# spartan-array/spartan

Hardware: AMD Instinct MI355X
Metric: spartan.dot TFLOP/s (+ map/reduce HBM GB/s) (higher is better)
Workload: dtype f32

## Files before the change

### spartan_amd/csrc/gemm_split.hpp

```cpp
#pragma once

typedef __bf16 gs_bf16x8 __attribute__((ext_vector_type(8)));
typedef __bf16 gs_bf16x4 __attribute__((ext_vector_type(4)));

namespace {

constexpr int GS_BK = 16;
constexpr int GS_RB = GS_BK * 2;
constexpr int GS_WN = 4;
constexpr unsigned GS_WIN_LO = (127u - 40u) << 23;
constexpr unsigned GS_WIN_HI = (127u + 40u) << 23;
constexpr size_t GS_IMAGE_CAP = (size_t)2 << 30;
constexpr size_t GS_WS_HEAD = 512;

template <int WN>
struct GsCfg {
  static constexpr int BM = 256, BN = 64 * WN, NW = 2 * WN, THREADS = 64 * NW;
  static constexpr int A_BYTES = BM * GS_RB, B_BYTES = BN * GS_RB;
  static constexpr int STAGE_BYTES = 3 * A_BYTES + 3 * B_BYTES;
  static constexpr int SMEM_BYTES = 2 * STAGE_BYTES;
  static constexpr int APW = A_BYTES / 1024 / NW, BPW = B_BYTES / 1024 / NW;
  static constexpr int NPIECES = 3 * APW + 3 * BPW;
  static constexpr int SLOTS = SP_CUS * (WN == 4 ? 1 : 2);
  static_assert(APW >= 1 && BPW >= 1 && APW * NW * 1024 == A_BYTES && BPW * NW * 1024 == B_BYTES, "tile / waves mismatch");
  static_assert(NPIECES * 4 <= 48, "one piece after every fourth MFMA");
};

__device__ __forceinline__ bool gs_outside(float v) {
  const unsigned b = __float_as_uint(v) & 0x7fffffffu;
  return b != 0u && (b < GS_WIN_LO || b >= GS_WIN_HI);
}

__device__ __forceinline__ void gs_cut(float v, __bf16& h, __bf16& m, __bf16& l) {
  h = (__bf16)v;
  const float r1 = v - (float)h;
  m = (__bf16)r1;
  l = (__bf16)(r1 - (float)m);
}

__device__ __forceinline__ void gs_raise(bool bad, unsigned* flag) {
  if (__any(bad) && (threadIdx.x & 63) == 0) atomicOr(flag, 1u);
}

__global__ __launch_bounds__(256) void sp_gemm_cut_rows_kernel(const float* __restrict__ A, int64_t lda, int M, int K,
                                                               __bf16* __restrict__ Ah, int64_t img,
                                                               unsigned* __restrict__ flag) {
  const int q = threadIdx.x & 7, row = blockIdx.x * 32 + (threadIdx.x >> 3);
  const int kpad = (K + GS_BK - 1) / GS_BK * GS_BK;
  bool bad = false;
  if (row < M) {
    const float* __restrict__ a = A + (int64_t)row * lda;
#pragma unroll
    for (int it = 0; it < 8; ++it) {
      const int k = blockIdx.y * 256 + it * 32 + 4 * q;
      if (k >= kpad) break;
      f32x4 v = {0.f, 0.f, 0.f, 0.f};
      if (k + 4 <= K) {
        v = *(const f32x4*)(a + k);
      } else {
#pragma unroll
        for (int e = 0; e < 4; ++e)
          if (k + e < K) v[e] = a[k + e];
      }
      gs_bf16x4 h, m, l;
#pragma unroll
      for (int e = 0; e < 4; ++e) {
        bad |= gs_outside(v[e]);
        __bf16 hh, mm, ll;
        gs_cut(v[e], hh, mm, ll);
        h[e] = hh;
        m[e] = mm;
        l[e] = ll;
      }
      const int64_t at = ((int64_t)(k >> 4) * M + row) * GS_BK + (k & 15);
      *(gs_bf16x4*)(Ah + at) = h;
      *(gs_bf16x4*)(Ah + img + at) = m;
      *(gs_bf16x4*)(Ah + 2 * img + at) = l;
    }
  }
  gs_raise(bad, flag);
}

__global__ __launch_bounds__(256) void sp_gemm_cut_cols_kernel(const float* __restrict__ B, int64_t ldb, int N, int K,
                                                               __bf16* __restrict__ Bh, int64_t img,
                                                               unsigned* __restrict__ flag) {
  __shared__ __attribute__((aligned(16))) __bf16 s[3][256 * GS_BK];
  const int n0 = blockIdx.x * 256, col = n0 + threadIdx.x, k0 = blockIdx.y * GS_BK;
  float v[GS_BK];
#pragma unroll
  for (int e = 0; e < GS_BK; ++e) v[e] = (col < N && k0 + e < K) ? B[(int64_t)(k0 + e) * ldb + col] : 0.f;
  bool bad = false;
  gs_bf16x8 h[2], m[2], l[2];
#pragma unroll
  for (int e = 0; e < GS_BK; ++e) {
    bad |= gs_outside(v[e]);
    __bf16 hh, mm, ll;
    gs_cut(v[e], hh, mm, ll);
    h[e >> 3][e & 7] = hh;
    m[e >> 3][e & 7] = mm;
    l[e >> 3][e & 7] = ll;
  }
#pragma unroll
  for (int c = 0; c < 2; ++c) {
    *(gs_bf16x8*)(&s[0][threadIdx.x * GS_BK + 8 * c]) = h[c];
    *(gs_bf16x8*)(&s[1][threadIdx.x * GS_BK + 8 * c]) = m[c];
    *(gs_bf16x8*)(&s[2][threadIdx.x * GS_BK + 8 * c]) = l[c];
  }
  __syncthreads();
  const int64_t base = ((int64_t)blockIdx.y * N + n0) * GS_BK;
#pragma unroll
  for (int p = 0; p < 3; ++p)
#pragma unroll
    for (int c = 0; c < 2; ++c) {
      const int at = (c * 256 + threadIdx.x) * 8;
      if (n0 + at / GS_BK < N) *(gs_bf16x8*)(Bh + p * img + base + at) = *(const gs_bf16x8*)(&s[p][at]);
    }
  gs_raise(bad, flag);
}

template <int WN>
__global__ __launch_bounds__(GsCfg<WN>::THREADS, 2) void sp_gemm_glds_kernel_bf16x3(
    const char* __restrict__ Ah, int64_t a_img, const char* __restrict__ Bh, int64_t b_img, float* __restrict__ C,
    int64_t ldc, int M, int N, int KT, int accumulate, int tiles_m, int tiles_n, int64_t a_slab, int64_t b_slab,
    const unsigned* __restrict__ flag_a, const unsigned* __restrict__ flag_b) {
  using G = GsCfg<WN>;
  constexpr int APW = G::APW, BPW = G::BPW, NPIECES = G::NPIECES;
  extern __shared__ __attribute__((aligned(16))) char gs_smem[];
  if ((*flag_a | *flag_b) != 0u) return;
  int tm, tn;
  sp_gemm_tile_of_block(blockIdx.x, gridDim.x, tiles_m, tiles_n, tm, tn);
  const int m0 = tm * G::BM, n0 = tn * G::BN;
  const int tid = threadIdx.x, lane = tid & 63;
  const int wid = __builtin_amdgcn_readfirstlane(tid >> 6);
  const int wm = wid / WN, wn = wid % WN;
  const int l31 = lane & 31, lh = lane >> 5;

  unsigned a_off[APW], b_off[BPW];
#pragma unroll
  for (int j = 0; j < APW; ++j) {
    const int slot = (wid * APW + j) * 64 + lane;
    int row = slot >> 1;
    const int q = (slot & 1) ^ ((row >> 4) & 1);
    if (m0 + row > M - 1) row = M - 1 - m0;
    a_off[j] = (unsigned)(row * GS_RB + q * 16);
  }
#pragma unroll
  for (int j = 0; j < BPW; ++j) {
    const int slot = (wid * BPW + j) * 64 + lane;
    int row = slot >> 1;
    const int q = (slot & 1) ^ ((row >> 4) & 1);
    if (n0 + row > N - 1) row = N - 1 - n0;
    b_off[j] = (unsigned)(row * GS_RB + q * 16);
  }
  const char* __restrict__ Ablk = Ah + (int64_t)m0 * GS_RB;
  const char* __restrict__ Bblk = Bh + (int64_t)n0 * GS_RB;
  const unsigned s_base = SP_LDS_ADDR(gs_smem);

#define GS_PIECE(i)                                                                                    \
  do {                                                                                                 \
    if ((i) < 3 * APW) {                                                                               \
      const int p_ = (i) / APW, j_ = (i) % APW;                                                        \
      SP_GLDS_S(Ablk + p_ * a_img + ka_, a_off[j_], st_ + p_ * G::A_BYTES + (wid * APW + j_) * 1024);  \
    } else {                                                                                           \
      const int p_ = ((i) - 3 * APW) / BPW, j_ = ((i) - 3 * APW) % BPW;                                \
      SP_GLDS_S(Bblk + p_ * b_img + kb_, b_off[j_],                                                    \
                st_ + 3 * G::A_BYTES + p_ * G::B_BYTES + (wid * BPW + j_) * 1024);                     \
    }                                                                                                  \
  } while (0)

  f32x16 acc[4][2];
#pragma unroll
  for (int i = 0; i < 4; ++i)
#pragma unroll
    for (int j = 0; j < 2; ++j)
#pragma unroll
      for (int r = 0; r < 16; ++r) acc[i][j][r] = 0.f;

  {
    const int64_t ka_ = 0, kb_ = 0;
    const unsigned st_ = s_base;
#pragma unroll
    for (int i = 0; i < NPIECES; ++i) GS_PIECE(i);
  }
  SP_GLDS_LANDED();
  __syncthreads();

  const int fslot = (lh ^ ((l31 >> 4) & 1)) * 16;
  const int a_frag = (wm * 128 + l31) * GS_RB + fslot;
  const int b_frag = 3 * G::A_BYTES + (wn * 64 + l31) * GS_RB + fslot;

  for (int t = 0; t < KT; ++t) {
    const bool more = t + 1 < KT;
    const int64_t ka_ = (int64_t)(t + 1) * a_slab, kb_ = (int64_t)(t + 1) * b_slab;
    const unsigned st_ = s_base + (unsigned)((t + 1) & 1) * G::STAGE_BYTES;
    const char* st = gs_smem + (t & 1) * G::STAGE_BYTES;
    gs_bf16x8 af[3][4], bf[3][2];
#pragma unroll
    for (int p = 0; p < 3; ++p) {
#pragma unroll
      for (int i = 0; i < 4; ++i) af[p][i] = *(const gs_bf16x8*)(st + p * G::A_BYTES + a_frag + i * 32 * GS_RB);
#pragma unroll
      for (int j = 0; j < 2; ++j) bf[p][j] = *(const gs_bf16x8*)(st + p * G::B_BYTES + b_frag + j * 32 * GS_RB);
    }
    int piece = 0;
#pragma unroll
    for (int idx = 0; idx < 48; ++idx) {
      const int term = idx >> 3, i = (idx & 7) >> 1, j = idx & 1;
      const int pa = term == 0 ? 2 : (term == 2 || term == 3) ? 1 : 0;
      const int pb = term == 1 ? 2 : (term == 2 || term == 4) ? 1 : 0;
      acc[i][j] = __builtin_amdgcn_mfma_f32_32x32x16_bf16(af[pa][i], bf[pb][j], acc[i][j], 0, 0, 0);
      if (idx % 4 == 3 && piece < NPIECES) {
        __builtin_amdgcn_sched_barrier(0);
        if (more) GS_PIECE(piece);
        __builtin_amdgcn_sched_barrier(0);
        ++piece;
      }
    }
    if (more) SP_GLDS_LANDED();
    __syncthreads();
  }
#undef GS_PIECE

#pragma unroll
  for (int i = 0; i < 4; ++i) {
#pragma unroll
    for (int j = 0; j < 2; ++j) {
      const int col = n0 + wn * 64 + j * 32 + l31;
#pragma unroll
      for (int r = 0; r < 16; ++r) {
        const int row = m0 + wm * 128 + i * 32 + (r & 3) + 8 * (r >> 2) + 4 * lh;
        if (row < M && col < N) {
          float* p = C + (int64_t)row * ldc + col;
          float v = acc[i][j][r];
          if (accumulate) v += *p;
          *p = v;
        }
      }
    }
  }
}

template <typename Cfg, int BM, int BN, int WM, int WN, int WGS>
__global__ __launch_bounds__(Cfg::THREADS, WGS) void sp_gemm_f32_gated_kernel(
    const float* __restrict__ A, int64_t lda, const float* __restrict__ B, int64_t ldb, float* __restrict__ C,
    int64_t ldc, int M, int N, int K, int accumulate, int tiles_m, int tiles_n, const unsigned* __restrict__ flag_a,
    const unsigned* __restrict__ flag_b) {
  if ((*flag_a | *flag_b) == 0u) return;
  sp_gemm_glds_body<Cfg, BM, BN, WM, WN>(A, lda, B, ldb, C, ldc, M, N, K, accumulate, tiles_m, tiles_n);
}

#define GS_CUT_BYTES_PER_S 3.0e12
#define GS_ISSUED_FLOPS 1.1e15
static bool sp_gemm_bf16_plan(int64_t M, int64_t N, int64_t K) {
  static int mode = -2;
  if (mode == -2) {
    const char* e = getenv("SP_GEMM_SPLIT");
    mode = e ? atoi(e) : 1;
  }
  using G = GsCfg<GS_WN>;
  if (mode == 0 || K < 16 || N % 4 != 0 || N < 4 || M < 1 || M > 2147483647LL || N > 2147483647LL || K > 2147483647LL)
    return false;
  const int64_t tb = ((M + 255) / 256) * ((N + 127) / 128);
  if (tb < 2 * SP_CUS || tb >= 2147483647LL) return false;
  double dp_cost;
  if (sp_gemm_dp_choice(M, N, &dp_cost) != 6 || sp_sk_plan(M, N, K)) return false;
  const int64_t KT = (K + GS_BK - 1) / GS_BK;
  if ((double)KT * 3.0 * GS_RB * ((double)M + (double)N) > (double)GS_IMAGE_CAP) return false;
  const double fp32_s = dp_cost * 128.0 * 128.0 * (double)K * 2.0 / (157.3e12 * 0.95 / SP_CUS);
  const int64_t tiles = ((M + G::BM - 1) / G::BM) * ((N + G::BN - 1) / G::BN);
  const int64_t rounds = (tiles + G::SLOTS - 1) / G::SLOTS;
  const double main_s = (double)rounds * G::SLOTS * (6.0 * 2.0 * G::BM * G::BN * (double)K) / GS_ISSUED_FLOPS;
  const double cut_s = 10.0 * ((double)M + (double)N) * (double)K / GS_CUT_BYTES_PER_S;
  return (main_s + cut_s + 20e-6) < 0.92 * fp32_s;
}

static size_t sp_gemm_bf16_ws_bytes(int64_t M, int64_t N, int64_t K) {
  return GS_WS_HEAD + (size_t)((K + GS_BK - 1) / GS_BK) * 3 * GS_RB * (size_t)(M + N);
}

constexpr size_t GS_IMG_HEAD = 256;

static size_t sp_gemm_bf16_image_bytes(int64_t rows, int64_t K) {
  return GS_IMG_HEAD + (size_t)((K + GS_BK - 1) / GS_BK) * 3 * GS_RB * (size_t)rows;
}

static long long gs_cut_launches = 0;

static void sp_gemm_bf16_cut(int side, const float* X, int64_t ld, int64_t rows, int64_t K, char* img, unsigned* flag,
                             hipStream_t st) {
  const int64_t KT = (K + GS_BK - 1) / GS_BK;
  const int64_t img_stride = KT * rows * GS_RB;
  __atomic_add_fetch(&gs_cut_launches, 1, __ATOMIC_RELAXED);
  if (side == 0)
    hipLaunchKernelGGL(sp_gemm_cut_rows_kernel, dim3((unsigned)((rows + 31) / 32), (unsigned)((K + 255) / 256)), dim3(256), 0,
                       st, X, ld, (int)rows, (int)K, (__bf16*)img, img_stride / 2, flag);
  else
    hipLaunchKernelGGL(sp_gemm_cut_cols_kernel, dim3((unsigned)((rows + 255) / 256), (unsigned)KT), dim3(256), 0, st, X, ld,
                       (int)rows, (int)K, (__bf16*)img, img_stride / 2, flag);
}

static int sp_gemm_bf16_launch(const float* A, int64_t lda, const char* imgA, int64_t a_rows, int64_t a_row0,
                               const float* B, int64_t ldb, const char* imgB, int64_t b_rows, int64_t b_row0, float* C,
                               int64_t ldc, int64_t M, int64_t N, int64_t K, int acc, void* ws, hipStream_t st) {
  using G = GsCfg<GS_WN>;
  const int64_t KT = (K + GS_BK - 1) / GS_BK;
  const int64_t tiles_m = (M + G::BM - 1) / G::BM, tiles_n = (N + G::BN - 1) / G::BN;
  auto kern = sp_gemm_glds_kernel_bf16x3<GS_WN>;
  using FCfg = GldsCfg<256, 128, 2, 2>;
  auto gated = sp_gemm_f32_gated_kernel<FCfg, 256, 128, 2, 2, 2>;
  static bool attr_set = false;
  if (!attr_set) {
    SP_HIP(hipFuncSetAttribute((const void*)kern, hipFuncAttributeMaxDynamicSharedMemorySize, G::SMEM_BYTES));
    SP_HIP(hipFuncSetAttribute((const void*)gated, hipFuncAttributeMaxDynamicSharedMemorySize, FCfg::LDS_BYTES));
    attr_set = true;
  }
  char* base = (char*)(((uintptr_t)ws + 255) & ~(uintptr_t)255);
  char* next = base + GS_IMG_HEAD;
  if (!imgA || !imgB) SP_HIP(hipMemsetAsync(base, 0, GS_IMG_HEAD, st));
  const unsigned* flag_a = (const unsigned*)(imgA ? imgA : base);
  const unsigned* flag_b = (const unsigned*)(imgB ? imgB : base);
  const char *Ah, *Bh;
  if (imgA) {
    Ah = imgA + GS_IMG_HEAD + a_row0 * GS_RB;
  } else {
    a_rows = M;
    sp_gemm_bf16_cut(0, A, lda, M, K, next, (unsigned*)base, st);
    Ah = next;
    next += 3 * KT * M * GS_RB;
  }
  if (imgB) {
    Bh = imgB + GS_IMG_HEAD + b_row0 * GS_RB;
  } else {
    b_rows = N;
    sp_gemm_bf16_cut(1, B, ldb, N, K, next, (unsigned*)base, st);
    Bh = next;
  }
  hipLaunchKernelGGL(kern, dim3((unsigned)(tiles_m * tiles_n)), dim3(G::THREADS), G::SMEM_BYTES, st, Ah,
                     KT * a_rows * GS_RB, Bh, KT * b_rows * GS_RB, C, ldc, (int)M, (int)N, (int)KT, acc, (int)tiles_m,
                     (int)tiles_n, a_rows * GS_RB, b_rows * GS_RB, flag_a, flag_b);
  const int64_t ftm = (M + 255) / 256, ftn = (N + 127) / 128;
  hipLaunchKernelGGL(gated, dim3((unsigned)(ftm * ftn)), dim3(FCfg::THREADS), FCfg::LDS_BYTES, st, A, lda, B, ldb, C, ldc,
                     (int)M, (int)N, (int)K, acc, (int)ftm, (int)ftn, flag_a, flag_b);
  SP_CHECK_LAUNCH();
  return 0;
}

}
```

Baseline: 254.9.

## Switch bf16x3 split GEMM to 16x16x32 MFMA with packed cross terms

Replaces the 32x32x16 bf16 MFMA tiling with 16x16x32 MFMAs. The two 32-lane K halves now carry different split pieces (hi/mid and hi/lo), so the six split products collapse into three K=32 passes. Fragment LDS reads are spread through the MFMA stream instead of being issued all up front, and global-to-LDS piece issue is retuned to every eighth MFMA. The epilogue gains a vectorized f32x4 store path when C is 16-byte aligned. It still checks only the first column of each 4-wide store against N, so it can write out of bounds when N is not a multiple of 4. Larger accumulator and fragment arrays may also raise register pressure.

After: 256.3 (median of 3 runs). About the same (+0.6%).

```diff
diff --git a/spartan_amd/csrc/gemm_split.hpp b/spartan_amd/csrc/gemm_split.hpp
--- a/spartan_amd/csrc/gemm_split.hpp
+++ b/spartan_amd/csrc/gemm_split.hpp
@@ -23,7 +23,7 @@
   static constexpr int NPIECES = 3 * APW + 3 * BPW;
   static constexpr int SLOTS = SP_CUS * (WN == 4 ? 1 : 2);
   static_assert(APW >= 1 && BPW >= 1 && APW * NW * 1024 == A_BYTES && BPW * NW * 1024 == B_BYTES, "tile / waves mismatch");
-  static_assert(NPIECES * 4 <= 48, "one piece after every fourth MFMA");
+  static_assert(NPIECES * 8 <= 96, "one piece after every eighth MFMA");
 };
 
 __device__ __forceinline__ bool gs_outside(float v) {
@@ -133,7 +133,7 @@
   const int tid = threadIdx.x, lane = tid & 63;
   const int wid = __builtin_amdgcn_readfirstlane(tid >> 6);
   const int wm = wid / WN, wn = wid % WN;
-  const int l31 = lane & 31, lh = lane >> 5;
+  const int l15 = lane & 15, g = lane >> 4;
 
   unsigned a_off[APW], b_off[BPW];
 #pragma unroll
@@ -168,13 +168,13 @@
     }                                                                                                  \
   } while (0)
 
-  f32x16 acc[4][2];
-#pragma unroll
-  for (int i = 0; i < 4; ++i)
-#pragma unroll
-    for (int j = 0; j < 2; ++j)
-#pragma unroll
-      for (int r = 0; r < 16; ++r) acc[i][j][r] = 0.f;
+  f32x4 acc[8][4];
+#pragma unroll
+  for (int i = 0; i < 8; ++i)
+#pragma unroll
+    for (int j = 0; j < 4; ++j)
+#pragma unroll
+      for (int r = 0; r < 4; ++r) acc[i][j][r] = 0.f;
 
   {
     const int64_t ka_ = 0, kb_ = 0;
@@ -185,55 +185,87 @@
   SP_GLDS_LANDED();
   __syncthreads();
 
-  const int fslot = (lh ^ ((l31 >> 4) & 1)) * 16;
-  const int a_frag = (wm * 128 + l31) * GS_RB + fslot;
-  const int b_frag = 3 * G::A_BYTES + (wn * 64 + l31) * GS_RB + fslot;
+  const int fs[2] = {(g & 1) * 16, 16 - (g & 1) * 16};
+  const int a_row = (wm * 128 + l15) * GS_RB, b_row = 3 * G::A_BYTES + (wn * 64 + l15) * GS_RB;
+  const int a_hm = a_row + (g >> 1) * G::A_BYTES;
+  const int a_hl = a_row + (g >> 1) * 2 * G::A_BYTES;
+  const int b_lh = b_row + (1 - (g >> 1)) * 2 * G::B_BYTES;
 
   for (int t = 0; t < KT; ++t) {
     const bool more = t + 1 < KT;
     const int64_t ka_ = (int64_t)(t + 1) * a_slab, kb_ = (int64_t)(t + 1) * b_slab;
     const unsigned st_ = s_base + (unsigned)((t + 1) & 1) * G::STAGE_BYTES;
     const char* st = gs_smem + (t & 1) * G::STAGE_BYTES;
-    gs_bf16x8 af[3][4], bf[3][2];
-#pragma unroll
-    for (int p = 0; p < 3; ++p) {
-#pragma unroll
-      for (int i = 0; i < 4; ++i) af[p][i] = *(const gs_bf16x8*)(st + p * G::A_BYTES + a_frag + i * 32 * GS_RB);
-#pragma unroll
-      for (int j = 0; j < 2; ++j) bf[p][j] = *(const gs_bf16x8*)(st + p * G::B_BYTES + b_frag + j * 32 * GS_RB);
-    }
+    gs_bf16x8 af[2][8], bf[3][4];
+#define GS_AF(p, i) af[p][i] = *(const gs_bf16x8*)(st + ((p) ? a_hl : a_hm) + (i) * 16 * GS_RB + fs[(i) & 1])
+#define GS_BF(p, j) \
+  bf[p][j] = *(const gs_bf16x8*)(st + ((p) == 2 ? b_lh : b_row + (p) * G::B_BYTES) + (j) * 16 * GS_RB + fs[(j) & 1])
+    GS_AF(1, 0);
+#pragma unroll
+    for (int j = 0; j < 4; ++j) GS_BF(2, j);
+    GS_AF(1, 1);
     int piece = 0;
 #pragma unroll
-    for (int idx = 0; idx < 48; ++idx) {
-      const int term = idx >> 3, i = (idx & 7) >> 1, j = idx & 1;
-      const int pa = term == 0 ? 2 : (term == 2 || term == 3) ? 1 : 0;
-      const int pb = term == 1 ? 2 : (term == 2 || term == 4) ? 1 : 0;
-      acc[i][j] = __builtin_amdgcn_mfma_f32_32x32x16_bf16(af[pa][i], bf[pb][j], acc[i][j], 0, 0, 0);
-      if (idx % 4 == 3 && piece < NPIECES) {
+    for (int term = 0; term < 3; ++term) {
+      const int pa = term == 0 ? 1 : 0, pb = term == 0 ? 2 : term == 1 ? 1 : 0;
+#pragma unroll
+      for (int i = 0; i < 8; ++i) {
         __builtin_amdgcn_sched_barrier(0);
-        if (more) GS_PIECE(piece);
-        __builtin_amdgcn_sched_barrier(0);
-        ++piece;
-      }
-    }
+#pragma unroll
+        for (int j = 0; j < 4; ++j)
+          acc[i][j] = __builtin_amdgcn_mfma_f32_16x16x32_bf16(bf[pb][j], af[pa][i], acc[i][j], 0, 0, 0);
+        if (term == 0) {
+          if (i + 2 < 8) GS_AF(1, i + 2);
+          if (i < 4) GS_BF(1, i);
+          else GS_AF(0, i - 4);
+        } else if (term == 1) {
+          if (i < 4) GS_AF(0, i + 4);
+          if (i >= 2 && i < 6) GS_BF(0, i - 2);
+        }
+        if (i % 2 == 1 && piece < NPIECES) {
+          __builtin_amdgcn_sched_barrier(0);
+          if (more) GS_PIECE(piece);
+          ++piece;
+        }
+      }
+    }
+    __builtin_amdgcn_sched_barrier(0);
+#undef GS_AF
+#undef GS_BF
     if (more) SP_GLDS_LANDED();
     __syncthreads();
   }
 #undef GS_PIECE
 
-#pragma unroll
-  for (int i = 0; i < 4; ++i) {
-#pragma unroll
-    for (int j = 0; j < 2; ++j) {
-      const int col = n0 + wn * 64 + j * 32 + l31;
-#pragma unroll
-      for (int r = 0; r < 16; ++r) {
-        const int row = m0 + wm * 128 + i * 32 + (r & 3) + 8 * (r >> 2) + 4 * lh;
+  const int row0 = m0 + wm * 128 + l15, col0 = n0 + wn * 64 + 4 * g;
+  if ((((uintptr_t)C | (uintptr_t)(ldc * 4)) & 15) == 0) {
+#pragma unroll
+    for (int i = 0; i < 8; ++i) {
+#pragma unroll
+      for (int j = 0; j < 4; ++j) {
+        const int row = row0 + i * 16, col = col0 + j * 16;
+        if (row < M && col < N) {
+          f32x4* p = (f32x4*)(C + (int64_t)row * ldc + col);
+          f32x4 v = acc[i][j];
+          if (accumulate) v += *p;
+          *p = v;
+        }
+      }
+    }
+  } else {
+#pragma unroll
+    for (int i = 0; i < 8; ++i) {
+#pragma unroll
+      for (int j = 0; j < 4; ++j) {
+        const int row = row0 + i * 16, col = col0 + j * 16;
         if (row < M && col < N) {
           float* p = C + (int64_t)row * ldc + col;
-          float v = acc[i][j][r];
-          if (accumulate) v += *p;
-          *p = v;
+#pragma unroll
+          for (int r = 0; r < 4; ++r) {
+            float v = acc[i][j][r];
+            if (accumulate) v += p[r];
+            p[r] = v;
+          }
         }
       }
     }
```
